# aipixel/GPS-Gaussian

Hardware: NVIDIA H100
Metric: novel_views_per_sec_1024sq_500kgauss (higher is better)
Workload: dtype f32

## Files before the change

### gps-gaussian_b200/_lib.py

```python
import ctypes as C
import os
import threading

import torch

_HERE = os.path.dirname(os.path.abspath(__file__))
LIB_PATH = os.path.join(_HERE, "lib", "libgpsg_sm90.so")


class GpsgError(RuntimeError):
    pass


class RasterSettings(C.Structure):
    _fields_ = [("image_height", C.c_int32), ("image_width", C.c_int32), ("tanfovx", C.c_float),
                ("tanfovy", C.c_float), ("bg", C.c_float * 3), ("scale_modifier", C.c_float),
                ("viewmatrix", C.c_float * 16), ("projmatrix", C.c_float * 16), ("sh_degree", C.c_int32),
                ("campos", C.c_float * 3), ("prefiltered", C.c_int32), ("debug", C.c_int32)]


class GeomView(C.Structure):
    _fields_ = [("depths", C.c_void_p), ("means2D", C.c_void_p), ("conic_opacity", C.c_void_p),
                ("tiles_touched", C.c_void_p), ("point_offsets", C.c_void_p)]


class BinningView(C.Structure):
    _fields_ = [("point_list_keys", C.c_void_p), ("point_list", C.c_void_p)]


class ImageView(C.Structure):
    _fields_ = [("final_T", C.c_void_p), ("n_contrib", C.c_void_p), ("ranges", C.c_void_p)]


ALLOC_FN = C.CFUNCTYPE(C.c_void_p, C.c_void_p, C.c_size_t)

if not os.path.exists(LIB_PATH):
    raise ImportError(
        f"{LIB_PATH} not found: the CUDA extension is not built. Run `python gps-gaussian_b200/build.py` "
        "(nvcc, sm_90a). There is deliberately no CPU / PyTorch fallback.")

lib = C.CDLL(LIB_PATH)

_vp, _i, _i64, _sz = C.c_void_p, C.c_int, C.c_int64, C.c_size_t
lib.gpsg_last_error.restype = C.c_char_p
lib.gpsg_last_error.argtypes = []
lib.gpsg_version.restype = _i
# ... 258 lines not shown
```

### gps-gaussian_b200/csrc/gpsg_capi.cu

```cuda
#include <cstdarg>
#include <cstdio>
#include <cstring>
#include <cstdlib>
#include "gpsg_internal.cuh"

namespace gpsg {

static thread_local char g_err[1024] = "";

void set_error(const char* fmt, ...) {
    va_list ap;
    va_start(ap, fmt);
    vsnprintf(g_err, sizeof(g_err), fmt, ap);
    va_end(ap);
}

Camera make_camera(const GpsgRasterSettings& s) {
    Camera c;
    memcpy(c.view, s.viewmatrix, sizeof(c.view));
    memcpy(c.proj, s.projmatrix, sizeof(c.proj));
    c.tanfovx = s.tanfovx;
    c.tanfovy = s.tanfovy;
    c.W = s.image_width;
    c.H = s.image_height;
// ... 37 lines not shown
GeomState GeomState::carve(void* base, int P, size_t scan_bytes) {
    return carve_geom((char*)align_up((size_t)base), P, scan_bytes, nullptr);
}

static BinningState carve_binning(char* p, size_t N, size_t sort_bytes, char** end) {
    BinningState b;
    const size_t n = N > 0 ? N : 1;
    b.slabA = take<float4>(p, n);
    b.slabB = take<float4>(p, n);
    b.slabC = take<float4>(p, n);
    b.keys = take<uint64_t>(p, n);
    b.vals = take<uint32_t>(p, n);
    b.keys_unsorted = take<uint64_t>(p, n);
    b.bucket = reinterpret_cast<uint2*>(b.keys_unsorted);
    b.vals_unsorted = take<uint32_t>(p, n);
    b.sort_temp = p;
    b.sort_temp_bytes = sort_bytes;
    p += align_up(sort_bytes);
    if (end) *end = p;
    return b;
}
size_t BinningState::required(size_t N, size_t sort_bytes) {
    char* end = nullptr;
    carve_binning(nullptr, N, sort_bytes, &end);
    return (size_t)(end - (char*)nullptr) + 256;
}
BinningState BinningState::carve(void* base, size_t N, size_t sort_bytes) {
    return carve_binning((char*)align_up((size_t)base), N, sort_bytes, nullptr);
}

static ImageState carve_image(char* p, int W, int H, char** end) {
    ImageState im;
    const size_t hw = (size_t)W * H;
    const size_t tiles = (size_t)((W + GPSG_TILE_X - 1) / GPSG_TILE_X) * ((H + GPSG_TILE_Y - 1) / GPSG_TILE_Y);
    im.final_T = take<float>(p, hw > 0 ? hw : 1);
    im.n_contrib = take<uint32_t>(p, hw > 0 ? hw : 1);
    im.ranges = take<uint2>(p, tiles > 0 ? tiles : 1);
    im.tile_count = take<uint32_t>(p, tiles > 0 ? tiles : 1);
    im.totals = take<uint32_t>(p, 64);
    im.tile_cursor = take<uint32_t>(p, tiles > 0 ? tiles : 1);
    im.big_tiles = take<uint32_t>(p, tiles > 0 ? tiles : 1);
    im.tile_order = take<uint32_t>(p, tiles > 0 ? tiles : 1);
    if (end) *end = p;
    return im;
}
size_t ImageState::required(int W, int H) {
    char* end = nullptr;
    carve_image(nullptr, W, H, &end);
    return (size_t)(end - (char*)nullptr) + 256;
}
ImageState ImageState::carve(void* base, int W, int H) { return carve_image((char*)align_up((size_t)base), W, H, nullptr); }


static GaussianSrc aos_src(const float* means3D, const float* scales, const float* rots, const float* opacities,
                           const float* colors, const float* cov3D_precomp) {
    GaussianSrc src;
    memset(&src, 0, sizeof(src));
// ... 125 lines not shown
    if (!bin_base) { set_error("binning allocator returned NULL"); return GPSG_E_ALLOC; }
    BinningState b = BinningState::carve(bin_base, N, sort_bytes);

    if (N > 0 && !radix_path) {
        { StageTimer t(ST_SCATTER, stream, 1); rc = launch_bucket_scatter(cam, P, radii, g, b, im, stream); }
        if (rc) return rc;
        { StageTimer t(ST_TILE_SORT, stream, max_count > 2048 ? 2 : 1); rc = launch_tile_sort_gather(cam, P, max_count, src, g, b, im, stream); }
        if (rc) return rc;
    } else if (N > 0) {
        { StageTimer t(ST_SCAN, stream, 2); rc = run_scan(g, P, stream); }
        if (rc) return rc;
        { StageTimer t(ST_DUPLICATE, stream, 1); rc = launch_duplicate(cam, P, radii, g, b, stream); }
        if (rc) return rc;
        { StageTimer t(ST_SORT, stream, 2 + (end_bit + 7) / 8); rc = run_sort(b, N, end_bit, stream); }
        if (rc) return rc;
        { StageTimer t(ST_GATHER, stream, 1); rc = launch_gather_ranges(cam, N, src, g, b, im, stream); }
        if (rc) return rc;
    }
    { StageTimer t(ST_RENDER_FWD, stream, 1); rc = launch_render_forward(cam, b, im, out_color, g.depths, out_depth, out_alpha, stream); }
    if (rc) return rc;
    if (s->debug) GPSG_CUDA(cudaStreamSynchronize(stream));
    return GPSG_OK;
}

static int check_fwd_flags(int flags) {
    GPSG_REQUIRE((flags & ~GPSG_FWD_ANTIALIAS) == 0, "unknown forward flag bits (GPSG_FWD_ANTIALIAS is the only flag)");
    return GPSG_OK;
}

static int check_aux_outputs(const float* out_depth, const float* out_alpha) {
    GPSG_REQUIRE((out_depth == nullptr) == (out_alpha == nullptr), "out_depth and out_alpha must both be NULL or both be set");
// ... 472 lines not shown
int gpsg_geom_view(const void* geom_buffer, int P, GpsgGeomView* out) {
    GPSG_REQUIRE(geom_buffer && out, "NULL pointer");
    GeomState g = GeomState::carve(const_cast<void*>(geom_buffer), P, 0);
    out->depths = g.depths;
    out->means2D = reinterpret_cast<const float*>(g.means2D);
    out->conic_opacity = reinterpret_cast<const float*>(g.conic_opacity);
    out->tiles_touched = g.tiles_touched;
    out->point_offsets = g.point_offsets;
    return GPSG_OK;
}
int gpsg_binning_view(const void* binning_buffer, int64_t num_rendered, GpsgBinningView* out) {
    GPSG_REQUIRE(binning_buffer && out && num_rendered >= 0, "bad argument");
    BinningState b = BinningState::carve(const_cast<void*>(binning_buffer), (size_t)num_rendered, 0);
    out->point_list_keys = b.keys;
    out->point_list = b.vals;
    return GPSG_OK;
}
int gpsg_image_view(const void* image_buffer, int W, int H, GpsgImageView* out) {
    GPSG_REQUIRE(image_buffer && out && W > 0 && H > 0, "bad argument");
    ImageState im = ImageState::carve(const_cast<void*>(image_buffer), W, H);
    out->final_T = im.final_T;
    out->n_contrib = im.n_contrib;
    out->ranges = reinterpret_cast<const uint32_t*>(im.ranges);
    return GPSG_OK;
}

int gpsg_corr_sampler_forward(int device, void* stream_, int dtype, int B, int H, int W1, int W2, const void* volume,
                              int64_t sb, int64_t sh, int64_t sw1, const float* coords, int64_t coords_sb, int radius,
                              void* out) {
    GPSG_REQUIRE(dtype == 0 || dtype == 1, "dtype must be 0 (fp32) or 1 (fp16)");
    GPSG_REQUIRE(B >= 0 && H >= 0 && W1 >= 0 && W2 >= 0 && radius >= 0 && radius <= 31, "bad shape / radius");
    if ((int64_t)B * H * W1 == 0) return GPSG_OK;
    GPSG_REQUIRE((volume || W2 == 0) && coords && out, "NULL pointer");
    GPSG_CUDA(cudaSetDevice(device));
    StageTimer t(ST_CORR_FWD, (cudaStream_t)stream_, 1);
    return launch_corr_fwd(dtype, B, H, W1, W2, volume, sb, sh, sw1, coords, coords_sb, radius, out,
                           (cudaStream_t)stream_);
}
// ... 132 lines not shown
```

### gps-gaussian_b200/csrc/gpsg_internal.cuh

```cuda
#pragma once
#include <cuda_runtime.h>
#include <stdint.h>
#include <stddef.h>
#include "../../include/gpsg.h"

#define GPSG_TILE_X 16
#define GPSG_TILE_Y 16
#define GPSG_TILE_PIX 256

namespace gpsg {

void set_error(const char* fmt, ...);

#define GPSG_CUDA(expr)                                                                         \
    do {                                                                                        \
        cudaError_t _e = (expr);                                                                \
        if (_e != cudaSuccess) {                                                                \
            gpsg::set_error("%s:%d: %s -> %s", __FILE__, __LINE__, #expr, cudaGetErrorString(_e)); \
            return GPSG_E_CUDA;                                                                 \
        }                                                                                       \
    } while (0)
#define GPSG_LAUNCH_CHECK() GPSG_CUDA(cudaGetLastError())
#define GPSG_REQUIRE(cond, msg)                                  \
    do {                                                         \
// ... 48 lines not shown
    x = xyz[0]; y = xyz[1]; z = xyz[2];
    const size_t S2 = (size_t)s.S2;
    sc[0] = s.scale[v][px]; sc[1] = s.scale[v][S2 + px]; sc[2] = s.scale[v][2 * S2 + px];
    q = make_float4(s.rot[v][px], s.rot[v][S2 + px], s.rot[v][2 * S2 + px], s.rot[v][3 * S2 + px]);
    op = s.opac[v][px];
    return true;
}
__device__ __forceinline__ void tile_rect(int grid_x, int grid_y, float2 p, int radius, int& rx0, int& ry0, int& rx1,
                                          int& ry1) {
    const float rad = (float)radius;
    rx0 = min(grid_x, max(0, (int)((p.x - rad) / (float)GPSG_TILE_X)));
    ry0 = min(grid_y, max(0, (int)((p.y - rad) / (float)GPSG_TILE_Y)));
    rx1 = min(grid_x, max(0, (int)((p.x + rad + (float)(GPSG_TILE_X - 1)) / (float)GPSG_TILE_X)));
    ry1 = min(grid_y, max(0, (int)((p.y + rad + (float)(GPSG_TILE_Y - 1)) / (float)GPSG_TILE_Y)));
}
__device__ __forceinline__ void src_color(const GaussianSrc& s, uint32_t id, float& r, float& g, float& b) {
    if (s.S2 == 0) { r = s.colors[3 * id]; g = s.colors[3 * id + 1]; b = s.colors[3 * id + 2]; return; }
    const int v = (int)id >= s.S2 ? 1 : 0;
    const size_t px = id - (uint32_t)(v * s.S2), S2 = (size_t)s.S2;
    r = s.img[v][px] * 0.5f + 0.5f; g = s.img[v][S2 + px] * 0.5f + 0.5f; b = s.img[v][2 * S2 + px] * 0.5f + 0.5f;
}
#endif

static inline size_t align_up(size_t v, size_t a = 256) { return (v + a - 1) / a * a; }

struct GeomState {
    float* depths;
    float2* means2D;
    float4* conic_opacity;
    float* rgb;
// ... 2 lines not shown
    uint32_t* point_offsets;
    void* scan_temp;
    size_t scan_temp_bytes;
    static size_t required(int P, size_t scan_temp_bytes);
    static GeomState carve(void* base, int P, size_t scan_temp_bytes);
};
struct BinningState {
    uint2* bucket;
    uint64_t* keys_unsorted;
    uint32_t* vals_unsorted;
    uint64_t* keys;
    uint32_t* vals;
    float4* slabA;
    float4* slabB;
    float4* slabC;
    void* sort_temp;
    size_t sort_temp_bytes;
    static size_t required(size_t N, size_t sort_temp_bytes);
    static BinningState carve(void* base, size_t N, size_t sort_temp_bytes);
};
struct ImageState {
    float* final_T;
    uint32_t* n_contrib;
    uint2* ranges;
    uint32_t* tile_count;
    uint32_t* tile_cursor;
    uint32_t* totals;
    uint32_t* big_tiles;
    uint32_t* tile_order;
    static size_t required(int W, int H);
    static ImageState carve(void* base, int W, int H);
};
constexpr int kFwdFlagsWord = 6;
size_t scan_temp_bytes(int P);
size_t sort_temp_bytes(size_t N, int end_bit);

int launch_preprocess(const Camera& cam, int P, const GaussianSrc& src, int32_t* radii, GeomState g, ImageState im,
                      uint32_t capacity, int fwd_flags, cudaStream_t stream);
int launch_mark_visible(int P, const float* means3D, const float* view16_host, uint8_t* present, cudaStream_t stream);
int run_scan(GeomState g, int P, cudaStream_t stream);
int launch_duplicate(const Camera& cam, int P, const int32_t* radii, GeomState g, BinningState b, cudaStream_t stream);
int run_sort(BinningState b, size_t N, int end_bit, cudaStream_t stream);
int launch_gather_ranges(const Camera& cam, size_t N, const GaussianSrc& src, GeomState g, BinningState b, ImageState im,
                         cudaStream_t stream);
// ... 72 lines not shown
```

### gps-gaussian_b200/csrc/raster_binning.cu

```cuda
#include <cub/cub.cuh>
#include "gpsg_internal.cuh"
#include "tile_scan.cuh"

namespace gpsg {

size_t scan_temp_bytes(int P) {
    size_t bytes = 0;
    cub::DeviceScan::InclusiveSum(nullptr, bytes, (uint32_t*)nullptr, (uint32_t*)nullptr, P > 0 ? P : 1);
    return bytes;
}

size_t sort_temp_bytes(size_t N, int end_bit) {
    size_t bytes = 0;
    cub::DeviceRadixSort::SortPairs(nullptr, bytes, (uint64_t*)nullptr, (uint64_t*)nullptr, (uint32_t*)nullptr,
                                    (uint32_t*)nullptr, (int64_t)(N > 0 ? N : 1), 0, end_bit);
    return bytes;
}

int run_scan(GeomState g, int P, cudaStream_t stream) {
    if (P <= 0) return GPSG_OK;
    size_t bytes = g.scan_temp_bytes;
    GPSG_CUDA(cub::DeviceScan::InclusiveSum(g.scan_temp, bytes, g.tiles_touched, g.point_offsets, P, stream));
    return GPSG_OK;
}
// ... 112 lines not shown
    if (!(co.w * 255.0f >= 1.0f)) {
        ex = ey = -3.0e38f;
    } else if (detc > 0.0f && co.x > 0.0f && co.z > 0.0f) {
        const float tau2 = 2.0f * __logf(co.w * 255.0f) * 1.0005f + 1e-4f;
        ex = sqrtf(tau2 * co.z / detc) * 1.0005f + 0.01f;
        ey = sqrtf(tau2 * co.x / detc) * 1.0005f + 0.01f;
        if (!(ex == ex) || !(ey == ey)) { ex = 3.0e38f; ey = 3.0e38f; }
    }
    A = make_float4(xy.x, xy.y, ex, ey);
    const float kL = 1.4426950408889634f;
    B = make_float4(-0.5f * kL * co.x, -kL * co.y, -0.5f * kL * co.z, co.w);
    C = make_float4(r, gg, bb, __uint_as_float(id));
}

constexpr int kSortThreads = 512;
constexpr int kSortCTAsPerSM = 3;
constexpr int kBigItems = (int)kMaxTileSort / kSortThreads;
template <int ITEMS>
struct TileSort {
    using BRS = cub::BlockRadixSort<uint32_t, kSortThreads, ITEMS, uint32_t, 4, false>;
    union Smem {
        typename BRS::TempStorage sort;
        unsigned long long keys[kSortThreads * ITEMS];
    };

    static constexpr int kMaxRun = 16;
    __device__ static void run(Smem& sm, uint32_t* flags, const uint2* __restrict__ src, int n, int id_bits, uint32_t tile,
                               size_t out0, const GaussianSrc& src_in, const GeomState& g, const BinningState& b) {
        uint32_t keys[ITEMS], ids[ITEMS];
        uint32_t dmin = ~0u, dmax = 0u;
#pragma unroll
        for (int k = 0; k < ITEMS; ++k) {
            const int i = k * kSortThreads + (int)threadIdx.x;
            const uint2 e = i < n ? src[i] : make_uint2(0u, 0u);
            ids[k] = e.x;
            keys[k] = e.y;
            if (i < n) { dmin = min(dmin, e.y); dmax = max(dmax, e.y); }
        }
        dmin = __reduce_min_sync(0xffffffffu, dmin);
        dmax = __reduce_max_sync(0xffffffffu, dmax);
        if (threadIdx.x == 0) { flags[0] = ~0u; flags[1] = 0u; flags[2] = 0u; }
        __syncthreads();
        if ((threadIdx.x & 31) == 0) { atomicMin(&flags[0], dmin); atomicMax(&flags[1], dmax); }
// ... 68 lines not shown
            if (r < n) {
                const unsigned long long v = sm.keys[r];
                const uint32_t id = (uint32_t)v;
                const size_t o = out0 + r;
                if (b.keys) {
                    b.keys[o] = tile_hi | (v >> 32);
                    b.vals[o] = id;
                }
                float4 A, B, C;
                slab_entry(id, src_in, g, A, B, C);
                b.slabA[o] = A;
                b.slabB[o] = B;
                b.slabC[o] = C;
            }
        }
    }
};

template <bool BIG>
__global__ void __launch_bounds__(kSortThreads, BIG ? 1 : kSortCTAsPerSM) tile_sort_gather_kernel(const GaussianSrc colors, GeomState g,
                                                                            BinningState b, ImageState im, int id_bits) {
    __shared__ uint32_t flags[4];
    if (im.totals[2]) return;
    if constexpr (BIG) {
        __shared__ typename TileSort<kBigItems>::Smem t16;
        const uint32_t nbig = im.totals[3];
        for (uint32_t k = blockIdx.x; k < nbig; k += gridDim.x) {
            const uint32_t tile = im.big_tiles[k];
            const uint2 range = im.ranges[tile];
            const int n = (int)(range.y - range.x);
            TileSort<kBigItems>::run(t16, flags, b.bucket + range.x, n, id_bits, tile, range.x, colors, g, b);
            __syncthreads();
        }
    } else {
        __shared__ union {
            typename TileSort<1>::Smem t1;
            typename TileSort<2>::Smem t2;
            typename TileSort<3>::Smem t3;
            typename TileSort<4>::Smem t4;
        } temp;
        const uint32_t tile = im.tile_order[blockIdx.x];
        const uint2 range = im.ranges[tile];
        const int n = (int)(range.y - range.x);
        if (n == 0 || n > (int)kBigTile) return;
        const uint2* __restrict__ src = b.bucket + range.x;
        if (n <= 512) TileSort<1>::run(temp.t1, flags, src, n, id_bits, tile, range.x, colors, g, b);
        else if (n <= 1024) TileSort<2>::run(temp.t2, flags, src, n, id_bits, tile, range.x, colors, g, b);
        else if (n <= 1536) TileSort<3>::run(temp.t3, flags, src, n, id_bits, tile, range.x, colors, g, b);
        else TileSort<4>::run(temp.t4, flags, src, n, id_bits, tile, range.x, colors, g, b);
    }
}

constexpr int kBigTileCTAs = 132;

int launch_tile_sort_gather(const Camera& cam, int P, uint32_t max_count, const GaussianSrc& colors, GeomState g,
                            BinningState b, ImageState im, cudaStream_t stream) {
    int id_bits = 1;
    while (id_bits < 32 && (1ll << id_bits) < (long long)P) ++id_bits;
    const int tiles = cam.grid_x * cam.grid_y;
    tile_sort_gather_kernel<false><<<tiles, kSortThreads, 0, stream>>>(colors, g, b, im, id_bits);
    GPSG_LAUNCH_CHECK();
    if (max_count > kBigTile) {
        tile_sort_gather_kernel<true><<<min(tiles, kBigTileCTAs), kSortThreads, 0, stream>>>(colors, g, b, im, id_bits);
        GPSG_LAUNCH_CHECK();
    }
    return GPSG_OK;
}

__global__ void __launch_bounds__(256) gather_ranges_kernel(size_t N, const GaussianSrc colors, GeomState g,
                                                            BinningState b, ImageState im) {
    const size_t i = (size_t)blockIdx.x * blockDim.x + threadIdx.x;
    if (i >= N) return;
    const uint64_t key = b.keys[i];
    const uint32_t tile = (uint32_t)(key >> 32);
    if (i == 0) {
        im.ranges[tile].x = 0;
    } else {
        const uint32_t prev = (uint32_t)(b.keys[i - 1] >> 32);
        if (prev != tile) {
            im.ranges[prev].y = (uint32_t)i;
            im.ranges[tile].x = (uint32_t)i;
        }
    }
    if (i == N - 1) im.ranges[tile].y = (uint32_t)N;
    const uint32_t id = b.vals[i];
    float4 A, B, C;
    slab_entry(id, colors, g, A, B, C);
    b.slabA[i] = A;
    b.slabB[i] = B;
    b.slabC[i] = C;
}

int launch_gather_ranges(const Camera& cam, size_t N, const GaussianSrc& colors, GeomState g, BinningState b, ImageState im,
                         cudaStream_t stream) {
    GPSG_CUDA(cudaMemsetAsync(im.ranges, 0, sizeof(uint2) * (size_t)cam.grid_x * cam.grid_y, stream));
    if (N == 0) return GPSG_OK;
    gather_ranges_kernel<<<(unsigned)((N + 255) / 256), 256, 0, stream>>>(N, colors, g, b, im);
    GPSG_LAUNCH_CHECK();
    return GPSG_OK;
}

}
```

### gps-gaussian_b200/csrc/raster_render.cu

```cuda
#include "gpsg_internal.cuh"
#include "slab_ring.cuh"

namespace gpsg {

struct f2p { float a, b; };
__device__ __forceinline__ f2p pk2(float lo, float hi) { return {lo, hi}; }
__device__ __forceinline__ void upk2(f2p v, float& lo, float& hi) { lo = v.a; hi = v.b; }
__device__ __forceinline__ f2p sub2(f2p x, f2p y) { return {__fsub_rn(x.a, y.a), __fsub_rn(x.b, y.b)}; }
__device__ __forceinline__ f2p mul2(f2p x, f2p y) { return {__fmul_rn(x.a, y.a), __fmul_rn(x.b, y.b)}; }
__device__ __forceinline__ f2p fma2(f2p x, f2p y, f2p z) { return {__fmaf_rn(x.a, y.a, z.a), __fmaf_rn(x.b, y.b, z.b)}; }

constexpr int kFwdChunk = 64;
constexpr int kFwdStages = 6;
constexpr int kFwdWarps = 4;

template <bool AUX>
__global__ void __launch_bounds__((kFwdWarps + 1) * 32, 8) render_forward_kernel(const __grid_constant__ Camera cam,
                                                                            const float4* __restrict__ slabA,
                                                                            const float4* __restrict__ slabB,
                                                                            const float4* __restrict__ slabC,
                                                                            const uint2* __restrict__ ranges, const uint32_t* __restrict__ tile_order,
                                                                            const uint32_t* __restrict__ status,
                                                                            float* __restrict__ final_T,
                                                                            uint32_t* __restrict__ n_contrib,
                                                                            float* __restrict__ out_color,
                                                                            const float* __restrict__ depths,
                                                                            float* __restrict__ out_depth,
                                                                            float* __restrict__ out_alpha) {
    __shared__ SlabRing<kFwdChunk, kFwdStages> ring;
    constexpr int kRows = AUX ? 6 : 5;
    __shared__ float4 qp[kFwdWarps][kRows][17];

    const int tid = threadIdx.x, lane = tid & 31, warp = tid >> 5;
    const int tile = (int)tile_order[blockIdx.x >> 1], half = blockIdx.x & 1;
    const int tile_y = tile / cam.grid_x, tile_x = tile - tile_y * cam.grid_x;
    const uint2 range = status[2] ? make_uint2(0u, 0u) : ranges[tile];
    const int total = (int)(range.y - range.x);
    const int nbatch = (total + kFwdChunk - 1) / kFwdChunk;

    if (tid == 0) ring_init(ring, kFwdWarps);
    for (int e = tid; e < kFwdWarps * kRows * 17; e += (kFwdWarps + 1) * 32) (&qp[0][0][0])[e] = make_float4(0.f, 0.f, 0.f, 0.f);
    __syncthreads();

    if (warp == kFwdWarps) {
        if (lane == 0)
            ring_produce(ring, nbatch, kFwdWarps, slabA, slabB, slabC,
                         [&](int b) { return (size_t)range.x + (size_t)b * kFwdChunk; },
                         [&](int b) { return min(kFwdChunk, total - b * kFwdChunk); });
        return;
    }
    const int bx0 = tile_x * GPSG_TILE_X + ((warp & 1) << 3);
    const int by0 = tile_y * GPSG_TILE_Y + (half << 3) + ((warp >> 1) << 2);
    const int px = bx0 + (lane & 7), py = by0 + (lane >> 3);
    const bool inside = px < cam.W && py < cam.H;
    const float pixfx = (float)px, pixfy = (float)py;
    const float wx0 = (float)bx0, wx1 = (float)(bx0 + 7), wy0 = (float)by0, wy1 = (float)(by0 + 3);

    float4 (*__restrict__ QP)[17] = qp[warp];
    const f2p pixfx2 = pk2(pixfx, pixfx), pixfy2 = pk2(pixfy, pixfy);
    const unsigned lt_mask = (1u << lane) - 1u;

    bool done = !inside;
    bool warp_done = __all_sync(0xffffffffu, done);
    if (warp_done && lane == 0) atomicAdd(&ring.done_warps, 1);
    float T = 1.0f, C0 = 0.0f, C1 = 0.0f, C2 = 0.0f, D = 0.0f;
    int last_contributor = 0;

    for (int b = 0; b < nbatch; ++b) {
        if (!ring_wait_full(ring, b, kFwdWarps)) break;
        if (!warp_done) {
            const int s = b % kFwdStages;
            const int n = min(kFwdChunk, total - b * kFwdChunk);
            const float4* __restrict__ SA = ring.A[s];
            const float4* __restrict__ SB = ring.B[s];
            const float4* __restrict__ SC = ring.C[s];
            const int posbase = b * kFwdChunk + 1;
            for (int base = 0; base < n; base += 32) {
                const int my = base + lane;
                bool hit = false;
                float4 a = make_float4(0.f, 0.f, 0.f, 0.f);
                if (my < n) {
                    a = SA[my];
                    hit = (a.x >= wx0 - a.z) && (a.x <= wx1 + a.z) && (a.y >= wy0 - a.w) && (a.y <= wy1 + a.w);
                }
                const unsigned m = __ballot_sync(0xffffffffu, hit);
                if (m) {
                    const int cnt = __popc(m);
                    if (hit) {
                        const int r = __popc(m & lt_mask);
                        const float4 q = SB[my];
                        const float4 c = SC[my];
                        float* base = reinterpret_cast<float*>(&QP[0][r >> 1]) + (r & 1);
                        constexpr int kS = 17 * 4;
                        base[0] = a.x;           base[2] = a.y;
                        base[kS] = q.x;          base[kS + 2] = q.y;
                        base[2 * kS] = q.z;      base[2 * kS + 2] = q.w;
                        base[3 * kS] = c.x;      base[3 * kS + 2] = c.y;
                        base[4 * kS] = c.z;      base[4 * kS + 2] = __int_as_float(posbase + my);
                        if constexpr (AUX) base[5 * kS] = depths[__float_as_uint(c.w)];
                    }
                    if (lane == 0 && (cnt & 1)) reinterpret_cast<float*>(&QP[2][cnt >> 1])[3] = 0.f;
                    __syncwarp();
#pragma unroll 4
                    for (int i = 0; i < cnt; i += 2) {
                        const int pr = i >> 1;
                        const float4 v0 = QP[0][pr], v1 = QP[1][pr], v2 = QP[2][pr], v3 = QP[3][pr], v4 = QP[4][pr];
                        float2 v5 = make_float2(0.f, 0.f);
                        if constexpr (AUX) v5 = *reinterpret_cast<const float2*>(&QP[5][pr]);
                        const f2p dx2 = sub2(pk2(v0.x, v0.y), pixfx2), dy2 = sub2(pk2(v0.z, v0.w), pixfy2);
                        const f2p t2 = fma2(pk2(v1.x, v1.y), dx2, mul2(pk2(v1.z, v1.w), dy2));
                        const f2p p2 = fma2(mul2(pk2(v2.x, v2.y), dy2), dy2, mul2(t2, dx2));
                        float pA, pB;
                        upk2(p2, pA, pB);
                        float aA, aB;
                        upk2(mul2(pk2(v2.z, v2.w), pk2(ex2_approx(pA), ex2_approx(pB))), aA, aB);
#pragma unroll
                        for (int u = 0; u < 2; ++u) {
                            const float p = u ? pB : pA;
                            const float alpha = fminf(0.99f, u ? aB : aA);
                            const bool valid = !done && !(p > 0.0f) && !(alpha < 1.0f / 255.0f);
                            const float test_T = T * (1.0f - alpha);
                            const bool stop = valid && (test_T < 0.0001f);
                            const bool upd = valid && !stop;
                            done = done || stop;
                            const float w = upd ? alpha * T : 0.0f;
                            C0 = fmaf(u ? v3.y : v3.x, w, C0);
                            C1 = fmaf(u ? v3.w : v3.z, w, C1);
                            C2 = fmaf(u ? v4.y : v4.x, w, C2);
                            if constexpr (AUX) D = fmaf(u ? v5.y : v5.x, w, D);
                            T = upd ? test_T : T;
                            last_contributor = upd ? __float_as_int(u ? v4.w : v4.z) : last_contributor;
                        }
                    }
                    __syncwarp();
                }
                if (__all_sync(0xffffffffu, done)) { warp_done = true; break; }
            }
            if (warp_done && lane == 0) atomicAdd(&ring.done_warps, 1);
        }
        ring_release(ring, b, lane);
    }

    if (inside) {
        const size_t HW = (size_t)cam.W * cam.H;
        const size_t pid = (size_t)py * cam.W + px;
        final_T[pid] = T;
        n_contrib[pid] = (uint32_t)last_contributor;
        out_color[pid] = fmaf(T, cam.bg[0], C0);
        out_color[HW + pid] = fmaf(T, cam.bg[1], C1);
        out_color[2 * HW + pid] = fmaf(T, cam.bg[2], C2);
        if constexpr (AUX) {
            out_depth[pid] = D;
            out_alpha[pid] = 1.0f - T;
        }
    }
}

int launch_render_forward(const Camera& cam, BinningState b, ImageState im, float* out_color, const float* depths,
                          float* out_depth, float* out_alpha, cudaStream_t stream) {
    const unsigned grid = 2u * (unsigned)(cam.grid_x * cam.grid_y);
    if (out_depth)
        render_forward_kernel<true><<<grid, (kFwdWarps + 1) * 32, 0, stream>>>(
            cam, b.slabA, b.slabB, b.slabC, im.ranges, im.tile_order, im.totals, im.final_T, im.n_contrib, out_color, depths,
            out_depth, out_alpha);
    else
        render_forward_kernel<false><<<grid, (kFwdWarps + 1) * 32, 0, stream>>>(
            cam, b.slabA, b.slabB, b.slabC, im.ranges, im.tile_order, im.totals, im.final_T, im.n_contrib, out_color, nullptr,
            nullptr, nullptr);
    GPSG_LAUNCH_CHECK();
    return GPSG_OK;
}

}
```

### gps-gaussian_b200/introspect.py

```python
import ctypes as C

import numpy as np
import torch

from . import _lib


def _sub(buf, ptr, nbytes, dtype):
    off = int(ptr) - buf.data_ptr()
    assert 0 <= off and off + nbytes <= buf.numel(), (off, nbytes, buf.numel())
    return buf[off:off + nbytes].view(dtype)


def make_settings(sc, debug=False):
    s = _lib.RasterSettings()
    s.image_height, s.image_width = int(sc["H"]), int(sc["W"])
    s.tanfovx, s.tanfovy = float(sc["tanfovx"]), float(sc["tanfovy"])
    s.bg[:] = [float(v) for v in np.asarray(sc["bg"]).reshape(3)]
    s.scale_modifier = float(sc.get("scale_modifier", 1.0))
    s.viewmatrix[:] = [float(v) for v in np.asarray(sc["view"], np.float32).reshape(16)]
    s.projmatrix[:] = [float(v) for v in np.asarray(sc["proj"], np.float32).reshape(16)]
    s.sh_degree = 3
    s.campos[:] = [float(v) for v in np.asarray(sc["campos"], np.float32).reshape(3)]
    s.prefiltered, s.debug = 0, int(debug)
# ... 43 lines not shown
        tiles = ((W + 15) // 16) * ((H + 15) // 16)
        st = dict(radii=self.radii, num_rendered=N)
        gv, bv, iv = _lib.GeomView(), _lib.BinningView(), _lib.ImageView()
        _lib.check(_lib.lib.gpsg_geom_view(C.c_void_p(geom.data_ptr()), P, C.byref(gv)), "gpsg_geom_view")
        _lib.check(_lib.lib.gpsg_image_view(C.c_void_p(image.data_ptr()), W, H, C.byref(iv)), "gpsg_image_view")
        if P > 0:
            st["depths"] = _sub(geom, gv.depths, 4 * P, torch.float32)
            st["means2D"] = _sub(geom, gv.means2D, 8 * P, torch.float32).view(P, 2)
            st["conic_opacity"] = _sub(geom, gv.conic_opacity, 16 * P, torch.float32).view(P, 4)
            st["tiles_touched"] = _sub(geom, gv.tiles_touched, 4 * P, torch.int32)
            st["point_offsets"] = _sub(geom, gv.point_offsets, 4 * P, torch.int32)
        if N > 0:
            _lib.check(_lib.lib.gpsg_binning_view(C.c_void_p(binning.data_ptr()), N, C.byref(bv)), "gpsg_binning_view")
            st["keys"] = _sub(binning, bv.point_list_keys, 8 * N, torch.int64)
            st["point_list"] = _sub(binning, bv.point_list, 4 * N, torch.int32)
        st["final_T"] = _sub(image, iv.final_T, 4 * H * W, torch.float32).view(H, W)
        st["n_contrib"] = _sub(image, iv.n_contrib, 4 * H * W, torch.int32).view(H, W)
        st["ranges"] = _sub(image, iv.ranges, 8 * tiles, torch.int32).view(tiles, 2)
        return st
```

### include/gpsg.h

```cpp
#ifndef GPSG_H
#define GPSG_H
#include <stddef.h>
#include <stdint.h>

#ifdef __cplusplus
extern "C" {
#endif

#if defined(__GNUC__)
#define GPSG_API __attribute__((visibility("default")))
#else
#define GPSG_API
#endif

#define GPSG_OK 0
#define GPSG_E_INVALID (-1)
#define GPSG_E_CUDA (-2)
#define GPSG_E_ALLOC (-3)
#define GPSG_E_CAPACITY (-4)

typedef struct GpsgRasterSettings {
    int32_t image_height;
    int32_t image_width;
    float tanfovx;
// ... 172 lines not shown
                                                    uint32_t* status_host, int flags);

GPSG_API int gpsg_mark_visible(int device, void* stream, int P, const float* means3D, const float* viewmatrix_host16,
                      uint8_t* present);

typedef struct GpsgGeomView {
    const float* depths;
    const float* means2D;
    const float* conic_opacity;
    const uint32_t* tiles_touched;
    const uint32_t* point_offsets;
} GpsgGeomView;
typedef struct GpsgBinningView {
    const uint64_t* point_list_keys;
    const uint32_t* point_list;
} GpsgBinningView;
typedef struct GpsgImageView {
    const float* final_T;
    const uint32_t* n_contrib;
    const uint32_t* ranges;
} GpsgImageView;
GPSG_API int gpsg_geom_view(const void* geom_buffer, int P, GpsgGeomView* out);
GPSG_API int gpsg_binning_view(const void* binning_buffer, int64_t num_rendered, GpsgBinningView* out);
GPSG_API int gpsg_image_view(const void* image_buffer, int W, int H, GpsgImageView* out);

GPSG_API int gpsg_corr_sampler_forward(int device, void* stream, int dtype, int B, int H, int W1, int W2, const void* volume,
                              int64_t sb, int64_t sh, int64_t sw1, const float* coords, int64_t coords_sb,
                              int radius, void* out);
GPSG_API int gpsg_corr_sampler_backward(int device, void* stream, int dtype, int B, int H, int W1, int W2,
                               const float* coords, int64_t coords_sb, const void* grad_out, int radius,
                               void* grad_volume);

GPSG_API int gpsg_corr_build_pyramid(int device, void* stream, int dtype, int B, int D, int H, int W1, int W2,
                                     const void* fmap1, const void* fmap2, void* const* vols, int levels);
GPSG_API int gpsg_corr_build_backward(int device, void* stream, int dtype, int B, int D, int H, int W1, int W2,
// ... 33 lines not shown
```

Before: 4735.

## Cull per-subblock Gaussian lists and render each tile via per-warp cp.async queues

After the per-tile sort, each tile's sorted Gaussians are filtered into eight 8x4-pixel sub-block lists using each Gaussian's bounding extent, and per-block counts are stored. The forward render kernel is restructured so each warp handles one sub-block, walking only that block's list with a double-buffered cp.async queue instead of a shared producer/consumer ring. This cuts wasted alpha evaluations for Gaussians that miss a sub-block, at the cost of an extra list-building pass, 8x list storage in the binning buffer, and an extra kernel on the radix path.

```diff
diff --git a/gps-gaussian_b200/_lib.py b/gps-gaussian_b200/_lib.py
--- a/gps-gaussian_b200/_lib.py
+++ b/gps-gaussian_b200/_lib.py
@@ -25,11 +25,11 @@
 
 
 class BinningView(C.Structure):
-    _fields_ = [("point_list_keys", C.c_void_p), ("point_list", C.c_void_p)]
+    _fields_ = [("point_list_keys", C.c_void_p), ("point_list", C.c_void_p), ("slabA", C.c_void_p), ("block_lists", C.c_void_p)]
 
 
 class ImageView(C.Structure):
-    _fields_ = [("final_T", C.c_void_p), ("n_contrib", C.c_void_p), ("ranges", C.c_void_p)]
+    _fields_ = [("final_T", C.c_void_p), ("n_contrib", C.c_void_p), ("ranges", C.c_void_p), ("block_counts", C.c_void_p)]
 
 
 ALLOC_FN = C.CFUNCTYPE(C.c_void_p, C.c_void_p, C.c_size_t)
diff --git a/gps-gaussian_b200/csrc/gpsg_capi.cu b/gps-gaussian_b200/csrc/gpsg_capi.cu
--- a/gps-gaussian_b200/csrc/gpsg_capi.cu
+++ b/gps-gaussian_b200/csrc/gpsg_capi.cu
@@ -75,6 +75,7 @@
     b.keys_unsorted = take<uint64_t>(p, n);
     b.bucket = reinterpret_cast<uint2*>(b.keys_unsorted);
     b.vals_unsorted = take<uint32_t>(p, n);
+    b.blk_list = take<uint32_t>(p, 8 * n);
     b.sort_temp = p;
     b.sort_temp_bytes = sort_bytes;
     p += align_up(sort_bytes);
@@ -102,6 +103,7 @@
     im.tile_cursor = take<uint32_t>(p, tiles > 0 ? tiles : 1);
     im.big_tiles = take<uint32_t>(p, tiles > 0 ? tiles : 1);
     im.tile_order = take<uint32_t>(p, tiles > 0 ? tiles : 1);
+    im.blk_count = take<uint32_t>(p, 8 * (tiles > 0 ? tiles : 1));
     if (end) *end = p;
     return im;
 }
@@ -257,7 +259,7 @@
         if (rc) return rc;
         { StageTimer t(ST_SORT, stream, 2 + (end_bit + 7) / 8); rc = run_sort(b, N, end_bit, stream); }
         if (rc) return rc;
-        { StageTimer t(ST_GATHER, stream, 1); rc = launch_gather_ranges(cam, N, src, g, b, im, stream); }
+        { StageTimer t(ST_GATHER, stream, 2); rc = launch_gather_ranges(cam, N, src, g, b, im, stream); }
         if (rc) return rc;
     }
     { StageTimer t(ST_RENDER_FWD, stream, 1); rc = launch_render_forward(cam, b, im, out_color, g.depths, out_depth, out_alpha, stream); }
@@ -760,6 +762,8 @@
     BinningState b = BinningState::carve(const_cast<void*>(binning_buffer), (size_t)num_rendered, 0);
     out->point_list_keys = b.keys;
     out->point_list = b.vals;
+    out->slabA = reinterpret_cast<const float*>(b.slabA);
+    out->block_lists = b.blk_list;
     return GPSG_OK;
 }
 int gpsg_image_view(const void* image_buffer, int W, int H, GpsgImageView* out) {
@@ -768,6 +772,7 @@
     out->final_T = im.final_T;
     out->n_contrib = im.n_contrib;
     out->ranges = reinterpret_cast<const uint32_t*>(im.ranges);
+    out->block_counts = im.blk_count;
     return GPSG_OK;
 }
 
diff --git a/gps-gaussian_b200/csrc/gpsg_internal.cuh b/gps-gaussian_b200/csrc/gpsg_internal.cuh
--- a/gps-gaussian_b200/csrc/gpsg_internal.cuh
+++ b/gps-gaussian_b200/csrc/gpsg_internal.cuh
@@ -86,6 +86,12 @@
     rx1 = min(grid_x, max(0, (int)((p.x + rad + (float)(GPSG_TILE_X - 1)) / (float)GPSG_TILE_X)));
     ry1 = min(grid_y, max(0, (int)((p.y + rad + (float)(GPSG_TILE_Y - 1)) / (float)GPSG_TILE_Y)));
 }
+__device__ __forceinline__ int fwd_block_col(int k) { return (k >> 1) & 1; }
+__device__ __forceinline__ int fwd_block_row(int k) { return ((k >> 2) << 1) + (k & 1); }
+__device__ __forceinline__ void fwd_block_origin(int tile_x, int tile_y, int k, int& bx0, int& by0) {
+    bx0 = tile_x * GPSG_TILE_X + (fwd_block_col(k) << 3);
+    by0 = tile_y * GPSG_TILE_Y + (fwd_block_row(k) << 2);
+}
 __device__ __forceinline__ void src_color(const GaussianSrc& s, uint32_t id, float& r, float& g, float& b) {
     if (s.S2 == 0) { r = s.colors[3 * id]; g = s.colors[3 * id + 1]; b = s.colors[3 * id + 2]; return; }
     const int v = (int)id >= s.S2 ? 1 : 0;
@@ -118,6 +124,7 @@
     float4* slabA;
     float4* slabB;
     float4* slabC;
+    uint32_t* blk_list;
     void* sort_temp;
     size_t sort_temp_bytes;
     static size_t required(size_t N, size_t sort_temp_bytes);
@@ -132,6 +139,7 @@
     uint32_t* totals;
     uint32_t* big_tiles;
     uint32_t* tile_order;
+    uint32_t* blk_count;
     static size_t required(int W, int H);
     static ImageState carve(void* base, int W, int H);
 };
diff --git a/gps-gaussian_b200/csrc/raster_binning.cu b/gps-gaussian_b200/csrc/raster_binning.cu
--- a/gps-gaussian_b200/csrc/raster_binning.cu
+++ b/gps-gaussian_b200/csrc/raster_binning.cu
@@ -150,7 +150,72 @@
 }
 
 constexpr int kSortThreads = 512;
+constexpr int kSortWarps = kSortThreads / 32;
 constexpr int kSortCTAsPerSM = 3;
+
+struct BlockLists {
+    uint32_t cnt[kSortWarps][8];
+    uint32_t off[kSortWarps][8];
+    uint32_t base[8];
+};
+
+__device__ __forceinline__ void build_block_lists(BlockLists& s, const float4* __restrict__ tileA, uint32_t n, int tile_x,
+                                                  int tile_y, uint32_t* __restrict__ list, uint32_t* __restrict__ count) {
+    const int lane = threadIdx.x & 31, warp = threadIdx.x >> 5;
+    const unsigned lt = (1u << lane) - 1u;
+    float wx0[2], wx1[2], wy0[4], wy1[4];
+#pragma unroll
+    for (int k = 0; k < 8; ++k) {
+        int bx0, by0;
+        fwd_block_origin(tile_x, tile_y, k, bx0, by0);
+        wx0[fwd_block_col(k)] = (float)bx0; wx1[fwd_block_col(k)] = (float)(bx0 + 7);
+        wy0[fwd_block_row(k)] = (float)by0; wy1[fwd_block_row(k)] = (float)(by0 + 3);
+    }
+    if (threadIdx.x < 8) s.base[threadIdx.x] = 0u;
+#pragma unroll 1
+    for (uint32_t c0 = 0; c0 < n; c0 += kSortThreads) {
+        const uint32_t r = c0 + threadIdx.x;
+        const bool valid = r < n;
+        const float4 a = valid ? tileA[r] : make_float4(0.f, 0.f, 0.f, 0.f);
+        bool hx[2], hy[4];
+#pragma unroll
+        for (int c = 0; c < 2; ++c) hx[c] = (a.x >= wx0[c] - a.z) && (a.x <= wx1[c] + a.z);
+#pragma unroll
+        for (int w = 0; w < 4; ++w) hy[w] = (a.y >= wy0[w] - a.w) && (a.y <= wy1[w] + a.w);
+        uint32_t hits = 0u;
+#pragma unroll
+        for (int k = 0; k < 8; ++k) {
+            const bool hit = valid && hx[fwd_block_col(k)] && hy[fwd_block_row(k)];
+            hits |= (uint32_t)hit << k;
+            const unsigned m = __ballot_sync(0xffffffffu, hit);
+            if (lane == k) s.cnt[warp][k] = __popc(m);
+        }
+        __syncthreads();
+        if (threadIdx.x < kSortWarps * 8) {
+            static_assert(kSortWarps == 16, "one 16-lane segment per block");
+            const int k = threadIdx.x >> 4, w = threadIdx.x & 15;
+            const uint32_t cw = s.cnt[w][k];
+            uint32_t incl = cw;
+#pragma unroll
+            for (int o = 1; o < 16; o <<= 1) {
+                const uint32_t u = __shfl_up_sync(0xffffffffu, incl, o, 16);
+                if (w >= o) incl += u;
+            }
+            const uint32_t b = s.base[k];
+            s.off[w][k] = b + incl - cw;
+            __syncwarp();
+            if (w == 15) s.base[k] = b + incl;
+        }
+        __syncthreads();
+#pragma unroll
+        for (int k = 0; k < 8; ++k) {
+            const unsigned m = __ballot_sync(0xffffffffu, (hits >> k) & 1u);
+            if ((hits >> k) & 1u) list[(size_t)k * n + s.off[warp][k] + __popc(m & lt)] = r;
+        }
+    }
+    if (threadIdx.x < 8) count[threadIdx.x] = s.base[threadIdx.x];
+}
+
 constexpr int kBigItems = (int)kMaxTileSort / kSortThreads;
 template <int ITEMS>
 struct TileSort {
@@ -161,8 +226,9 @@
     };
 
     static constexpr int kMaxRun = 16;
-    __device__ static void run(Smem& sm, uint32_t* flags, const uint2* __restrict__ src, int n, int id_bits, uint32_t tile,
-                               size_t out0, const GaussianSrc& src_in, const GeomState& g, const BinningState& b) {
+    __device__ static void run(Smem& sm, uint32_t* flags, BlockLists& bl, const uint2* __restrict__ src, int n, int id_bits,
+                               uint32_t tile, int grid_x, size_t out0, const GaussianSrc& src_in, const GeomState& g,
+                               const BinningState& b, uint32_t* __restrict__ blk_count) {
         uint32_t keys[ITEMS], ids[ITEMS];
         uint32_t dmin = ~0u, dmax = 0u;
 #pragma unroll
@@ -261,13 +327,18 @@
                 b.slabC[o] = C;
             }
         }
+        const int tile_y = (int)tile / grid_x;
+        build_block_lists(bl, b.slabA + out0, (uint32_t)n, (int)tile - tile_y * grid_x, tile_y, b.blk_list + 8 * out0,
+                          blk_count + 8 * (size_t)tile);
     }
 };
 
 template <bool BIG>
 __global__ void __launch_bounds__(kSortThreads, BIG ? 1 : kSortCTAsPerSM) tile_sort_gather_kernel(const GaussianSrc colors, GeomState g,
-                                                                            BinningState b, ImageState im, int id_bits) {
+                                                                            BinningState b, ImageState im, int id_bits,
+                                                                            int grid_x) {
     __shared__ uint32_t flags[4];
+    __shared__ BlockLists bl;
     if (im.totals[2]) return;
     if constexpr (BIG) {
         __shared__ typename TileSort<kBigItems>::Smem t16;
@@ -276,7 +347,8 @@
             const uint32_t tile = im.big_tiles[k];
             const uint2 range = im.ranges[tile];
             const int n = (int)(range.y - range.x);
-            TileSort<kBigItems>::run(t16, flags, b.bucket + range.x, n, id_bits, tile, range.x, colors, g, b);
+            TileSort<kBigItems>::run(t16, flags, bl, b.bucket + range.x, n, id_bits, tile, grid_x, range.x, colors, g, b,
+                                     im.blk_count);
             __syncthreads();
         }
     } else {
@@ -291,10 +363,10 @@
         const int n = (int)(range.y - range.x);
         if (n == 0 || n > (int)kBigTile) return;
         const uint2* __restrict__ src = b.bucket + range.x;
-        if (n <= 512) TileSort<1>::run(temp.t1, flags, src, n, id_bits, tile, range.x, colors, g, b);
-        else if (n <= 1024) TileSort<2>::run(temp.t2, flags, src, n, id_bits, tile, range.x, colors, g, b);
-        else if (n <= 1536) TileSort<3>::run(temp.t3, flags, src, n, id_bits, tile, range.x, colors, g, b);
-        else TileSort<4>::run(temp.t4, flags, src, n, id_bits, tile, range.x, colors, g, b);
+        if (n <= 512) TileSort<1>::run(temp.t1, flags, bl, src, n, id_bits, tile, grid_x, range.x, colors, g, b, im.blk_count);
+        else if (n <= 1024) TileSort<2>::run(temp.t2, flags, bl, src, n, id_bits, tile, grid_x, range.x, colors, g, b, im.blk_count);
+        else if (n <= 1536) TileSort<3>::run(temp.t3, flags, bl, src, n, id_bits, tile, grid_x, range.x, colors, g, b, im.blk_count);
+        else TileSort<4>::run(temp.t4, flags, bl, src, n, id_bits, tile, grid_x, range.x, colors, g, b, im.blk_count);
     }
 }
 
@@ -305,10 +377,11 @@
     int id_bits = 1;
     while (id_bits < 32 && (1ll << id_bits) < (long long)P) ++id_bits;
     const int tiles = cam.grid_x * cam.grid_y;
-    tile_sort_gather_kernel<false><<<tiles, kSortThreads, 0, stream>>>(colors, g, b, im, id_bits);
+    tile_sort_gather_kernel<false><<<tiles, kSortThreads, 0, stream>>>(colors, g, b, im, id_bits, cam.grid_x);
     GPSG_LAUNCH_CHECK();
     if (max_count > kBigTile) {
-        tile_sort_gather_kernel<true><<<min(tiles, kBigTileCTAs), kSortThreads, 0, stream>>>(colors, g, b, im, id_bits);
+        tile_sort_gather_kernel<true><<<min(tiles, kBigTileCTAs), kSortThreads, 0, stream>>>(colors, g, b, im, id_bits,
+                                                                                             cam.grid_x);
         GPSG_LAUNCH_CHECK();
     }
     return GPSG_OK;
@@ -338,13 +411,27 @@
     b.slabC[i] = C;
 }
 
+__global__ void __launch_bounds__(kSortThreads) block_lists_kernel(int grid_x, BinningState b, ImageState im) {
+    __shared__ BlockLists bl;
+    const uint32_t tile = blockIdx.x;
+    const uint2 range = im.ranges[tile];
+    const uint32_t n = range.y - range.x;
+    if (n == 0) return;
+    const int tile_y = (int)tile / grid_x;
+    build_block_lists(bl, b.slabA + range.x, n, (int)tile - tile_y * grid_x, tile_y, b.blk_list + 8 * (size_t)range.x,
+                      im.blk_count + 8 * (size_t)tile);
+}
+
 int launch_gather_ranges(const Camera& cam, size_t N, const GaussianSrc& colors, GeomState g, BinningState b, ImageState im,
                          cudaStream_t stream) {
-    GPSG_CUDA(cudaMemsetAsync(im.ranges, 0, sizeof(uint2) * (size_t)cam.grid_x * cam.grid_y, stream));
+    const int tiles = cam.grid_x * cam.grid_y;
+    GPSG_CUDA(cudaMemsetAsync(im.ranges, 0, sizeof(uint2) * (size_t)tiles, stream));
     if (N == 0) return GPSG_OK;
     gather_ranges_kernel<<<(unsigned)((N + 255) / 256), 256, 0, stream>>>(N, colors, g, b, im);
     GPSG_LAUNCH_CHECK();
-    return GPSG_OK;
-}
-
-}
+    block_lists_kernel<<<tiles, kSortThreads, 0, stream>>>(cam.grid_x, b, im);
+    GPSG_LAUNCH_CHECK();
+    return GPSG_OK;
+}
+
+}
diff --git a/gps-gaussian_b200/csrc/raster_render.cu b/gps-gaussian_b200/csrc/raster_render.cu
--- a/gps-gaussian_b200/csrc/raster_render.cu
+++ b/gps-gaussian_b200/csrc/raster_render.cu
@@ -10,16 +10,75 @@
 __device__ __forceinline__ f2p mul2(f2p x, f2p y) { return {__fmul_rn(x.a, y.a), __fmul_rn(x.b, y.b)}; }
 __device__ __forceinline__ f2p fma2(f2p x, f2p y, f2p z) { return {__fmaf_rn(x.a, y.a, z.a), __fmaf_rn(x.b, y.b, z.b)}; }
 
-constexpr int kFwdChunk = 64;
-constexpr int kFwdStages = 6;
-constexpr int kFwdWarps = 4;
+constexpr int kFwdWarps = 2;
+constexpr int kFwdCTAsPerTile = 8 / kFwdWarps;
+constexpr int kFwdQ = 32;
+static_assert(kFwdWarps == 1 || kFwdWarps == 2 || kFwdWarps == 4, "a CTA holds 1, 2 or 4 of a tile's 8 blocks");
 
 template <bool AUX>
-__global__ void __launch_bounds__((kFwdWarps + 1) * 32, 8) render_forward_kernel(const __grid_constant__ Camera cam,
+struct FwdQueue {
+    float4 A[2][kFwdQ], B[2][kFwdQ], C[2][kFwdQ];
+    uint32_t pos[2][kFwdQ];
+    float z[2][AUX ? kFwdQ : 1];
+};
+
+struct FwdPixel {
+    float T = 1.0f, C0 = 0.0f, C1 = 0.0f, C2 = 0.0f, D = 0.0f;
+    uint32_t last = 0;
+    bool done;
+};
+
+template <bool AUX>
+__device__ __forceinline__ void fwd_eval_pair(const float4& a0, const float4& a1, const float4& b0, const float4& b1,
+                                              const float4& c0, const float4& c1, uint2 pos, float2 z, f2p pixfx2, f2p pixfy2,
+                                              FwdPixel& px) {
+    const f2p dx2 = sub2(pk2(a0.x, a1.x), pixfx2), dy2 = sub2(pk2(a0.y, a1.y), pixfy2);
+    const f2p t2 = fma2(pk2(b0.x, b1.x), dx2, mul2(pk2(b0.y, b1.y), dy2));
+    const f2p p2 = fma2(mul2(pk2(b0.z, b1.z), dy2), dy2, mul2(t2, dx2));
+    float pA, pB;
+    upk2(p2, pA, pB);
+    float aA, aB;
+    upk2(mul2(pk2(b0.w, b1.w), pk2(ex2_approx(pA), ex2_approx(pB))), aA, aB);
+#pragma unroll
+    for (int u = 0; u < 2; ++u) {
+        const float p = u ? pB : pA;
+        const float alpha = fminf(0.99f, u ? aB : aA);
+        const bool valid = !px.done && !(p > 0.0f) && !(alpha < 1.0f / 255.0f);
+        const float test_T = px.T * (1.0f - alpha);
+        const bool stop = valid && (test_T < 0.0001f);
+        const bool upd = valid && !stop;
+        px.done = px.done || stop;
+        const float w = upd ? alpha * px.T : 0.0f;
+        const float4& c = u ? c1 : c0;
+        px.C0 = fmaf(c.x, w, px.C0);
+        px.C1 = fmaf(c.y, w, px.C1);
+        px.C2 = fmaf(c.z, w, px.C2);
+        if constexpr (AUX) px.D = fmaf(u ? z.y : z.x, w, px.D);
+        px.T = upd ? test_T : px.T;
+        px.last = upd ? (u ? pos.y : pos.x) : px.last;
+    }
+}
+
+__device__ __forceinline__ void cp_async16(void* smem, const void* gmem) {
+    asm volatile("cp.async.cg.shared.global [%0], [%1], 16;" ::"r"((uint32_t)__cvta_generic_to_shared(smem)), "l"(gmem)
+                 : "memory");
+}
+__device__ __forceinline__ void cp_async4(void* smem, const void* gmem) {
+    asm volatile("cp.async.ca.shared.global [%0], [%1], 4;" ::"r"((uint32_t)__cvta_generic_to_shared(smem)), "l"(gmem)
+                 : "memory");
+}
+__device__ __forceinline__ void cp_async_commit() { asm volatile("cp.async.commit_group;" ::: "memory"); }
+__device__ __forceinline__ void cp_async_wait1() { asm volatile("cp.async.wait_group 1;" ::: "memory"); }
+__device__ __forceinline__ void cp_async_wait_all() { asm volatile("cp.async.wait_all;" ::: "memory"); }
+
+template <bool AUX>
+__global__ void __launch_bounds__(kFwdWarps * 32, 32 / kFwdWarps) render_forward_kernel(const __grid_constant__ Camera cam,
                                                                             const float4* __restrict__ slabA,
                                                                             const float4* __restrict__ slabB,
                                                                             const float4* __restrict__ slabC,
+                                                                            const uint32_t* __restrict__ blk_list,
                                                                             const uint2* __restrict__ ranges, const uint32_t* __restrict__ tile_order,
+                                                                            const uint32_t* __restrict__ blk_count,
                                                                             const uint32_t* __restrict__ status,
                                                                             float* __restrict__ final_T,
                                                                             uint32_t* __restrict__ n_contrib,
@@ -27,146 +86,109 @@
                                                                             const float* __restrict__ depths,
                                                                             float* __restrict__ out_depth,
                                                                             float* __restrict__ out_alpha) {
-    __shared__ SlabRing<kFwdChunk, kFwdStages> ring;
-    constexpr int kRows = AUX ? 6 : 5;
-    __shared__ float4 qp[kFwdWarps][kRows][17];
-
-    const int tid = threadIdx.x, lane = tid & 31, warp = tid >> 5;
-    const int tile = (int)tile_order[blockIdx.x >> 1], half = blockIdx.x & 1;
+    __shared__ FwdQueue<AUX> queues[kFwdWarps];
+    const int lane = threadIdx.x & 31, warp = threadIdx.x >> 5;
+    const int tile = (int)tile_order[blockIdx.x / kFwdCTAsPerTile];
+    const int blk = (int)(blockIdx.x % kFwdCTAsPerTile) * kFwdWarps + warp;
     const int tile_y = tile / cam.grid_x, tile_x = tile - tile_y * cam.grid_x;
-    const uint2 range = status[2] ? make_uint2(0u, 0u) : ranges[tile];
-    const int total = (int)(range.y - range.x);
-    const int nbatch = (total + kFwdChunk - 1) / kFwdChunk;
-
-    if (tid == 0) ring_init(ring, kFwdWarps);
-    for (int e = tid; e < kFwdWarps * kRows * 17; e += (kFwdWarps + 1) * 32) (&qp[0][0][0])[e] = make_float4(0.f, 0.f, 0.f, 0.f);
-    __syncthreads();
-
-    if (warp == kFwdWarps) {
-        if (lane == 0)
-            ring_produce(ring, nbatch, kFwdWarps, slabA, slabB, slabC,
-                         [&](int b) { return (size_t)range.x + (size_t)b * kFwdChunk; },
-                         [&](int b) { return min(kFwdChunk, total - b * kFwdChunk); });
-        return;
-    }
-    const int bx0 = tile_x * GPSG_TILE_X + ((warp & 1) << 3);
-    const int by0 = tile_y * GPSG_TILE_Y + (half << 3) + ((warp >> 1) << 2);
+    int bx0, by0;
+    fwd_block_origin(tile_x, tile_y, blk, bx0, by0);
     const int px = bx0 + (lane & 7), py = by0 + (lane >> 3);
     const bool inside = px < cam.W && py < cam.H;
-    const float pixfx = (float)px, pixfy = (float)py;
-    const float wx0 = (float)bx0, wx1 = (float)(bx0 + 7), wy0 = (float)by0, wy1 = (float)(by0 + 3);
+    const uint2 range = status[2] ? make_uint2(0u, 0u) : ranges[tile];
+    const uint32_t n = range.y - range.x;
+    const int cnt = n ? (int)blk_count[8 * tile + blk] : 0;
 
-    float4 (*__restrict__ QP)[17] = qp[warp];
-    const f2p pixfx2 = pk2(pixfx, pixfx), pixfy2 = pk2(pixfy, pixfy);
-    const unsigned lt_mask = (1u << lane) - 1u;
-
-    bool done = !inside;
-    bool warp_done = __all_sync(0xffffffffu, done);
-    if (warp_done && lane == 0) atomicAdd(&ring.done_warps, 1);
-    float T = 1.0f, C0 = 0.0f, C1 = 0.0f, C2 = 0.0f, D = 0.0f;
-    int last_contributor = 0;
-
-    for (int b = 0; b < nbatch; ++b) {
-        if (!ring_wait_full(ring, b, kFwdWarps)) break;
-        if (!warp_done) {
-            const int s = b % kFwdStages;
-            const int n = min(kFwdChunk, total - b * kFwdChunk);
-            const float4* __restrict__ SA = ring.A[s];
-            const float4* __restrict__ SB = ring.B[s];
-            const float4* __restrict__ SC = ring.C[s];
-            const int posbase = b * kFwdChunk + 1;
-            for (int base = 0; base < n; base += 32) {
-                const int my = base + lane;
-                bool hit = false;
-                float4 a = make_float4(0.f, 0.f, 0.f, 0.f);
-                if (my < n) {
-                    a = SA[my];
-                    hit = (a.x >= wx0 - a.z) && (a.x <= wx1 + a.z) && (a.y >= wy0 - a.w) && (a.y <= wy1 + a.w);
-                }
-                const unsigned m = __ballot_sync(0xffffffffu, hit);
-                if (m) {
-                    const int cnt = __popc(m);
-                    if (hit) {
-                        const int r = __popc(m & lt_mask);
-                        const float4 q = SB[my];
-                        const float4 c = SC[my];
-                        float* base = reinterpret_cast<float*>(&QP[0][r >> 1]) + (r & 1);
-                        constexpr int kS = 17 * 4;
-                        base[0] = a.x;           base[2] = a.y;
-                        base[kS] = q.x;          base[kS + 2] = q.y;
-                        base[2 * kS] = q.z;      base[2 * kS + 2] = q.w;
-                        base[3 * kS] = c.x;      base[3 * kS + 2] = c.y;
-                        base[4 * kS] = c.z;      base[4 * kS + 2] = __int_as_float(posbase + my);
-                        if constexpr (AUX) base[5 * kS] = depths[__float_as_uint(c.w)];
-                    }
-                    if (lane == 0 && (cnt & 1)) reinterpret_cast<float*>(&QP[2][cnt >> 1])[3] = 0.f;
-                    __syncwarp();
-#pragma unroll 4
-                    for (int i = 0; i < cnt; i += 2) {
-                        const int pr = i >> 1;
-                        const float4 v0 = QP[0][pr], v1 = QP[1][pr], v2 = QP[2][pr], v3 = QP[3][pr], v4 = QP[4][pr];
-                        float2 v5 = make_float2(0.f, 0.f);
-                        if constexpr (AUX) v5 = *reinterpret_cast<const float2*>(&QP[5][pr]);
-                        const f2p dx2 = sub2(pk2(v0.x, v0.y), pixfx2), dy2 = sub2(pk2(v0.z, v0.w), pixfy2);
-                        const f2p t2 = fma2(pk2(v1.x, v1.y), dx2, mul2(pk2(v1.z, v1.w), dy2));
-                        const f2p p2 = fma2(mul2(pk2(v2.x, v2.y), dy2), dy2, mul2(t2, dx2));
-                        float pA, pB;
-                        upk2(p2, pA, pB);
-                        float aA, aB;
-                        upk2(mul2(pk2(v2.z, v2.w), pk2(ex2_approx(pA), ex2_approx(pB))), aA, aB);
-#pragma unroll
-                        for (int u = 0; u < 2; ++u) {
-                            const float p = u ? pB : pA;
-                            const float alpha = fminf(0.99f, u ? aB : aA);
-                            const bool valid = !done && !(p > 0.0f) && !(alpha < 1.0f / 255.0f);
-                            const float test_T = T * (1.0f - alpha);
-                            const bool stop = valid && (test_T < 0.0001f);
-                            const bool upd = valid && !stop;
-                            done = done || stop;
-                            const float w = upd ? alpha * T : 0.0f;
-                            C0 = fmaf(u ? v3.y : v3.x, w, C0);
-                            C1 = fmaf(u ? v3.w : v3.z, w, C1);
-                            C2 = fmaf(u ? v4.y : v4.x, w, C2);
-                            if constexpr (AUX) D = fmaf(u ? v5.y : v5.x, w, D);
-                            T = upd ? test_T : T;
-                            last_contributor = upd ? __float_as_int(u ? v4.w : v4.z) : last_contributor;
-                        }
-                    }
-                    __syncwarp();
-                }
-                if (__all_sync(0xffffffffu, done)) { warp_done = true; break; }
+    FwdPixel pix;
+    pix.done = !inside;
+    if (cnt > 0 && !__all_sync(0xffffffffu, pix.done)) {
+        FwdQueue<AUX>& q = queues[warp];
+        const uint32_t* __restrict__ list = blk_list + 8 * (size_t)range.x + (size_t)blk * n;
+        const float4* __restrict__ tA = slabA + range.x;
+        const float4* __restrict__ tB = slabB + range.x;
+        const float4* __restrict__ tC = slabC + range.x;
+        const f2p pixfx2 = pk2((float)px, (float)px), pixfy2 = pk2((float)py, (float)py);
+        auto fetch = [&](int c, int buf, uint32_t p) {
+            const int m = min(kFwdQ, cnt - c);
+            if (lane < m) {
+                cp_async16(&q.A[buf][lane], tA + p);
+                cp_async16(&q.B[buf][lane], tB + p);
+                cp_async16(&q.C[buf][lane], tC + p);
+                q.pos[buf][lane] = p + 1u;
+            } else if (lane == m && (m & 1)) {
+                const float4 zero = make_float4(0.f, 0.f, 0.f, 0.f);
+                q.A[buf][lane] = zero; q.B[buf][lane] = zero; q.C[buf][lane] = zero;
+                q.pos[buf][lane] = 0u;
+                if constexpr (AUX) q.z[buf][lane] = 0.f;
             }
-            if (warp_done && lane == 0) atomicAdd(&ring.done_warps, 1);
+        };
+        auto fetch_z = [&](int c, int buf, uint32_t id) {
+            if (lane < cnt - c) cp_async4(&q.z[buf][lane], depths + id);
+        };
+        uint32_t p = lane < cnt ? list[lane] : 0u;
+        uint32_t id = 0u;
+        fetch(0, 0, p);
+        cp_async_commit();
+        if constexpr (AUX) {
+            if (lane < cnt) id = __float_as_uint(tC[p].w);
+            fetch_z(0, 0, id);
+            cp_async_commit();
         }
-        ring_release(ring, b, lane);
+        p = lane + kFwdQ < cnt ? list[lane + kFwdQ] : 0u;
+        for (int c = 0, buf = 0; c < cnt; c += kFwdQ, buf ^= 1) {
+            const bool more = c + kFwdQ < cnt;
+            if (more) {
+                fetch(c + kFwdQ, buf ^ 1, p);
+                if constexpr (AUX) { if (lane < cnt - c - kFwdQ) id = __float_as_uint(tC[p].w); }
+                if (c + 2 * kFwdQ + lane < cnt) p = list[c + 2 * kFwdQ + lane];
+            }
+            cp_async_commit();
+            cp_async_wait1();
+            __syncwarp();
+            const int m = min(kFwdQ, cnt - c);
+#pragma unroll 2
+            for (int i = 0; i < m; i += 2) {
+                float2 z = make_float2(0.f, 0.f);
+                if constexpr (AUX) z = *reinterpret_cast<const float2*>(&q.z[buf][i]);
+                fwd_eval_pair<AUX>(q.A[buf][i], q.A[buf][i + 1], q.B[buf][i], q.B[buf][i + 1], q.C[buf][i], q.C[buf][i + 1],
+                                   *reinterpret_cast<const uint2*>(&q.pos[buf][i]), z, pixfx2, pixfy2, pix);
+            }
+            __syncwarp();
+            if (__all_sync(0xffffffffu, pix.done)) break;
+            if constexpr (AUX) {
+                if (more) fetch_z(c + kFwdQ, buf ^ 1, id);
+                cp_async_commit();
+            }
+        }
+        cp_async_wait_all();
     }
 
     if (inside) {
         const size_t HW = (size_t)cam.W * cam.H;
         const size_t pid = (size_t)py * cam.W + px;
-        final_T[pid] = T;
-        n_contrib[pid] = (uint32_t)last_contributor;
-        out_color[pid] = fmaf(T, cam.bg[0], C0);
-        out_color[HW + pid] = fmaf(T, cam.bg[1], C1);
-        out_color[2 * HW + pid] = fmaf(T, cam.bg[2], C2);
+        final_T[pid] = pix.T;
+        n_contrib[pid] = pix.last;
+        out_color[pid] = fmaf(pix.T, cam.bg[0], pix.C0);
+        out_color[HW + pid] = fmaf(pix.T, cam.bg[1], pix.C1);
+        out_color[2 * HW + pid] = fmaf(pix.T, cam.bg[2], pix.C2);
         if constexpr (AUX) {
-            out_depth[pid] = D;
-            out_alpha[pid] = 1.0f - T;
+            out_depth[pid] = pix.D;
+            out_alpha[pid] = 1.0f - pix.T;
         }
     }
 }
 
 int launch_render_forward(const Camera& cam, BinningState b, ImageState im, float* out_color, const float* depths,
                           float* out_depth, float* out_alpha, cudaStream_t stream) {
-    const unsigned grid = 2u * (unsigned)(cam.grid_x * cam.grid_y);
+    const unsigned grid = (unsigned)kFwdCTAsPerTile * (unsigned)(cam.grid_x * cam.grid_y);
     if (out_depth)
-        render_forward_kernel<true><<<grid, (kFwdWarps + 1) * 32, 0, stream>>>(
-            cam, b.slabA, b.slabB, b.slabC, im.ranges, im.tile_order, im.totals, im.final_T, im.n_contrib, out_color, depths,
-            out_depth, out_alpha);
+        render_forward_kernel<true><<<grid, kFwdWarps * 32, 0, stream>>>(
+            cam, b.slabA, b.slabB, b.slabC, b.blk_list, im.ranges, im.tile_order, im.blk_count, im.totals, im.final_T,
+            im.n_contrib, out_color, depths, out_depth, out_alpha);
     else
-        render_forward_kernel<false><<<grid, (kFwdWarps + 1) * 32, 0, stream>>>(
-            cam, b.slabA, b.slabB, b.slabC, im.ranges, im.tile_order, im.totals, im.final_T, im.n_contrib, out_color, nullptr,
-            nullptr, nullptr);
+        render_forward_kernel<false><<<grid, kFwdWarps * 32, 0, stream>>>(
+            cam, b.slabA, b.slabB, b.slabC, b.blk_list, im.ranges, im.tile_order, im.blk_count, im.totals, im.final_T,
+            im.n_contrib, out_color, nullptr, nullptr, nullptr);
     GPSG_LAUNCH_CHECK();
     return GPSG_OK;
 }
diff --git a/gps-gaussian_b200/introspect.py b/gps-gaussian_b200/introspect.py
--- a/gps-gaussian_b200/introspect.py
+++ b/gps-gaussian_b200/introspect.py
@@ -81,7 +81,10 @@
             _lib.check(_lib.lib.gpsg_binning_view(C.c_void_p(binning.data_ptr()), N, C.byref(bv)), "gpsg_binning_view")
             st["keys"] = _sub(binning, bv.point_list_keys, 8 * N, torch.int64)
             st["point_list"] = _sub(binning, bv.point_list, 4 * N, torch.int32)
+            st["slabA"] = _sub(binning, bv.slabA, 16 * N, torch.float32).view(N, 4)
+            st["block_lists"] = _sub(binning, bv.block_lists, 32 * N, torch.int32)
         st["final_T"] = _sub(image, iv.final_T, 4 * H * W, torch.float32).view(H, W)
         st["n_contrib"] = _sub(image, iv.n_contrib, 4 * H * W, torch.int32).view(H, W)
         st["ranges"] = _sub(image, iv.ranges, 8 * tiles, torch.int32).view(tiles, 2)
+        st["block_counts"] = _sub(image, iv.block_counts, 32 * tiles, torch.int32).view(tiles, 8)
         return st
diff --git a/include/gpsg.h b/include/gpsg.h
--- a/include/gpsg.h
+++ b/include/gpsg.h
@@ -210,11 +210,14 @@
 typedef struct GpsgBinningView {
     const uint64_t* point_list_keys;
     const uint32_t* point_list;
+    const float* slabA;
+    const uint32_t* block_lists;
 } GpsgBinningView;
 typedef struct GpsgImageView {
     const float* final_T;
     const uint32_t* n_contrib;
     const uint32_t* ranges;
+    const uint32_t* block_counts;
 } GpsgImageView;
 GPSG_API int gpsg_geom_view(const void* geom_buffer, int P, GpsgGeomView* out);
 GPSG_API int gpsg_binning_view(const void* binning_buffer, int64_t num_rendered, GpsgBinningView* out);
```

Result: faster. 5079 (median of 6 runs) (+7.3%).
